# SUTD-MDQS/QILaplace.jl

Measured on AMD Instinct MI355X. Metric: MPO×MPS site-contractions/sec + max |coeff err|, n=24 χ_s=64 χ_c=128, higher is better.
Workload: dtype f64; 1 GPU; zt_n24_chi64_D128; sites=48, mps_bonds_max=64, mpo_bonds_max=128, parallelism=replicas x1 (one signal per GPU), ranks_reported_by_collective_backend=1

## Files before the change

### qilaplace.jl_amd/csrc/qil_internal.h

```cpp
#pragma once

#include <hip/hip_runtime.h>
#include <hip/hip_complex.h>

#include <cstdint>
#include <cstdio>
#include <cstring>
#include <functional>
#include <map>
#include <condition_variable>
#include <mutex>
#include <set>
#include <string>
#include <vector>

#include "qilaplace_hip.h"
#include "qilaplace_hip_testing.h"

#include <atomic>

struct qil_lds_grant {
    static constexpr int kDevices = 64;
    std::atomic<size_t> bytes[kDevices] = {};
    hipError_t ensure(int device, const void* fn, size_t want) {
// ... 145 lines not shown
        if (ctx) ctx->chains.erase(this);
    }
    int64_t n() const { return (int64_t)site.size(); }
    int64_t site_elems(int64_t i) const {
        return dims[i] * (phys_rank == 1 ? 2 : 4) * dims[i + 1];
    }
    size_t site_bytes(int64_t i) const { return (size_t)site_elems(i) * qil_elem_size(dtype); }
};
struct qil_mps : qil_chain {};
struct qil_mpo : qil_chain {};

int qil_chain_alloc(qil_context* ctx, qil_chain* c, int64_t n, int dtype, int paired, int phys_rank,
                    const int64_t* bond_dims, const int64_t* site_ids);
int qil_chain_release(qil_chain* c);
void qil_chain_bind(qil_chain* c, qil_context* ctx);
int qil_chain_set_site(qil_chain* c, int64_t i, void* p, int64_t dl, int64_t dr);
void qil_chain_adopt(qil_chain* c, int64_t i, void* p);

unsigned qil_fail_count();
struct qil_call_scope {
    qil_context* ctx;
    uint64_t serial0;
    unsigned fails0;
    explicit qil_call_scope(qil_context* c);
    ~qil_call_scope();
    qil_call_scope(const qil_call_scope&) = delete;
    qil_call_scope& operator=(const qil_call_scope&) = delete;
};

int qil_dev_right_envs(const struct qil_mps* psi, const char* verb, void** Rall, std::vector<long long>& roff, double* log_norm2);

int qil_dev_gemm(qil_context* ctx, int dtype, int opA, int opB, int64_t m, int64_t n, int64_t k,
                 const void* A, int64_t lda, const void* B, int64_t ldb, void* C, int64_t ldc);
int qil_dev_gemm_skinny(qil_context* ctx, int dtype, int opA, int opB, int64_t m, int64_t n, int64_t k,
                        const void* A, int64_t lda, const void* B, int64_t ldb, void* C, int64_t ldc);
struct qil_gemm_batch {
    int64_t count = 1;
    int64_t a_bs = 0, b_bs = 0, c_bs = 0;
    const uint8_t* b_sel = nullptr;
    int64_t b_sel_step = 0, b_sel_stride = 0;
};
int qil_dev_gemm_batched(qil_context* ctx, int dtype, int opA, int opB, int64_t m, int64_t n, int64_t k,
                         const void* A, int64_t lda, const void* B, int64_t ldb, void* C, int64_t ldc,
                         const qil_gemm_batch* batch);
struct qil_gemm_problem {
    const void* A;
    const void* B;
    void* C;
    int m, n, k;
    int lda, ldb, ldc;
    int tile_begin;
    int pad;
};
int qil_dev_gemm_grouped(qil_context* ctx, int dtype, std::vector<qil_gemm_problem>& probs);
bool qil_dev_gemm_grouped_fits(size_t nproblems);
int qil_check_pair(const char* verb, const struct qil_mps* phi, const struct qil_mps* psi);
int qil_sum_compress_impl(qil_context* ctx, const struct qil_mps* const* terms, int64_t nb, const double* w, int odt,
                          int64_t maxdim, double tol, int sweeps, int64_t zip_maxdim, struct qil_mps** out);
int qil_dev_diag_abs2(qil_context* ctx, int dtype, const void* R, int64_t ldr, int64_t n, double* host_out);
int qil_dev_transpose(qil_context* ctx, int dtype, int conj, int64_t m, int64_t n, const void* A, int64_t lda,
                      void* At, int64_t ldt);
int qil_dev_svd(qil_context* ctx, int dtype, int64_t m, int64_t n, void* A, int64_t lda, void* U,
                int64_t ldu, double* S_host, void* Vh, int64_t ldvh, double negligible_rel = 0.0);
int qil_dev_svd_left(qil_context* ctx, int dtype, int64_t p, int64_t q, void* B, int64_t ldb, void* Uiso, int64_t ldu,
                     double* S_host, void* SVh, int64_t ldsvh, double negligible_rel, int* handled, double cert_cutoff = 0.0,
                     double deflate = 0.0);
int qil_dev_qr_certified(qil_context* ctx, int dtype, int64_t m, int64_t n, const void* A, int64_t lda, double cutoff, void* Qout,
                         void* Rout, bool* certified);
// ... 14 lines not shown
```

### qilaplace.jl_amd/csrc/qil_linalg.hip

```cpp
#include <algorithm>
#include <chrono>
#include <cmath>
#include <cstring>
#include <numeric>
#include <utility>

#include "qil_internal.h"
#include "qil_launch.h"
#include "qil_device_utils.h"

namespace {

using namespace qil_dev;

constexpr int GK = 16;
#ifndef QIL_GEMM_GAUSS
#define QIL_GEMM_GAUSS 1
#endif
#ifndef QIL_GEMM_PAD
#define QIL_GEMM_PAD 2
#endif
constexpr int GPAD = QIL_GEMM_PAD;
typedef double d4 __attribute__((ext_vector_type(4)));

__device__ __forceinline__ void put_plane(double* S0, double* S1, int off, double v) {
    S0[off] = v;
    (void)S1;
}
__device__ __forceinline__ void put_plane(double* S0, double* S1, int off, c64 v) {
    S0[off] = v.re;
    S1[off] = v.im;
}
__device__ __forceinline__ double maybe_conj(double v, int) { return v; }
__device__ __forceinline__ c64 maybe_conj(c64 v, int cj) { return cj ? c64{v.re, -v.im} : v; }

template <class T, int BM, int BN, int WM, int WN, bool PIPE, bool ARC, bool BKC, int GKT = GK, int DEEP = 0>
__device__ __forceinline__ void gemm_mfma_body(const uint3 blockIdx, const uint3 gridDim, long long m, long long n, long long k_total,
                                                 const T* __restrict__ A, long long a_rs, long long a_ks, int conjA,
                                                 const T* __restrict__ B, long long b_ks, long long b_cs, int conjB,
                                                 T* __restrict__ C, long long ldc, long long kchunk,
                                                 long long cstride, int tiles_m, int tiles_n, int col_fastest,
                                                 long long a_bs, long long b_bs, long long c_bs,
                                                 const int* __restrict__ cmap, int cmap_blk,
                                                 const uint8_t* __restrict__ b_sel, long long b_sel_step,
                                                 long long b_sel_stride, int subtract) {
    constexpr bool CX = sizeof(T) == 16;
    constexpr int NP = CX ? 2 : 1;
    constexpr int LA = BM + GPAD, LB = BN + GPAD;
    constexpr int NBUF = PIPE ? 2 : 1;
    constexpr int TM = WM / 16, TN = WN / 16;
    constexpr int EA = BM * GKT / 256, EB = BN * GKT / 256;
    static_assert((BM / WM) * (BN / WN) == 4, "4 waves per workgroup");
    extern __shared__ __attribute__((aligned(16))) char gemm_smem[];
    double* As = reinterpret_cast<double*>(gemm_smem);
    double* Bs = As + NBUF * NP * GKT * LA;
    const int tid = threadIdx.x;
    const int lane = tid & 63, wave = tid >> 6;
    const int wr = (wave % (BM / WM)) * WM, wc = (wave / (BM / WM)) * WN;
    const int l15 = lane & 15, l4 = lane >> 4;
    int tile = blockIdx.x;
    if (col_fastest & 2) tile = (tile % 8) * (tiles_m * tiles_n / 8) + tile / 8;
    int tm, tn;
    if (col_fastest & 1) {
        tn = tile % tiles_n;
        tm = tile / tiles_n;
    } else {
        tm = tile % tiles_m;
        tn = tile / tiles_m;
    }
    const long long row0 = (long long)tm * BM, col0 = (long long)tn * BN;
    const long long kbeg = (long long)blockIdx.z * kchunk;
    const long long kend = min(k_total, kbeg + kchunk);
    A += (long long)blockIdx.y * a_bs;
    B += (long long)blockIdx.y * b_bs;
    if (b_sel) B += (long long)b_sel[(long long)blockIdx.y * b_sel_step] * b_sel_stride;
    C += (long long)blockIdx.z * cstride + (long long)blockIdx.y * c_bs;
    if (cmap) cmap += (long long)blockIdx.y * (n / cmap_blk);

    d4 rr[TM][TN], ii[CX ? TM : 1][CX ? TN : 1], ri[CX ? TM : 1][CX ? TN : 1];
#pragma unroll
    for (int a = 0; a < TM; ++a)
#pragma unroll
        for (int b = 0; b < TN; ++b) {
            rr[a][b] = d4{0, 0, 0, 0};
            if (CX) {
                ii[a][b] = d4{0, 0, 0, 0};
                ri[a][b] = d4{0, 0, 0, 0};
            }
        }
    constexpr bool a_rows_contig = ARC, b_k_contig = BKC;
    T ra[EA], rb[EB];
    const T* pa[EA];
    const T* pb[EB];
    int ka[EA], kb[EB], sa[EA], sb[EB];
#pragma unroll
    for (int e = 0; e < EA; ++e) {
        const int idx = tid + 256 * e;
        const int i = a_rows_contig ? idx % BM : idx / GKT;
        const int kk = a_rows_contig ? idx / BM : idx % GKT;
        const long long gr = row0 + i;
        ka[e] = kk;
        sa[e] = kk * LA + i;
        pa[e] = A + min(gr, m - 1) * a_rs + (kbeg + kk) * a_ks;
    }
#pragma unroll
    for (int e = 0; e < EB; ++e) {
        const int idx = tid + 256 * e;
        const int kk = b_k_contig ? idx % GKT : idx / BN;
        const int j = b_k_contig ? idx / GKT : idx % BN;
        const long long gc = col0 + j;
// ... 10 lines not shown
                pa[e] += a_step;
            }
#pragma unroll
            for (int e = 0; e < EB; ++e) {
                rb[e] = *pb[e];
                pb[e] += b_step;
            }
        } else {
#pragma unroll
            for (int e = 0; e < EA; ++e) ra[e] = *((k0 + ka[e] < kend) ? pa[e] : A);
#pragma unroll
            for (int e = 0; e < EB; ++e) rb[e] = *((k0 + kb[e] < kend) ? pb[e] : B);
        }
    };
    auto load_tile = [&](long long k0) { load_tile_into(ra, rb, k0); };
    auto store_tile_from = [&](const T(&ra)[EA], const T(&rb)[EB], int buf, long long k0) {
        double* a0 = As + (buf * NP) * GKT * LA;
        double* b0 = Bs + (buf * NP) * GKT * LB;
        if (k0 + GKT <= kend) {
#pragma unroll
            for (int e = 0; e < EA; ++e) put_plane(a0, a0 + GKT * LA, sa[e], maybe_conj(ra[e], conjA));
#pragma unroll
            for (int e = 0; e < EB; ++e) put_plane(b0, b0 + GKT * LB, sb[e], maybe_conj(rb[e], conjB));
        } else {
#pragma unroll
            for (int e = 0; e < EA; ++e)
                put_plane(a0, a0 + GKT * LA, sa[e], (k0 + ka[e] < kend) ? maybe_conj(ra[e], conjA) : T{});
#pragma unroll
            for (int e = 0; e < EB; ++e)
                put_plane(b0, b0 + GKT * LB, sb[e], (k0 + kb[e] < kend) ? maybe_conj(rb[e], conjB) : T{});
        }
    };
    auto store_tile = [&](int buf, long long k0) { store_tile_from(ra, rb, buf, k0); };
    auto mfma_tile = [&](int buf) {
        const double* a0 = As + (buf * NP) * GKT * LA;
        const double* b0 = Bs + (buf * NP) * GKT * LB;
#pragma unroll
        for (int kk = 0; kk < GKT; kk += 4) {
            double are[TM], aim[TM], bre[TN], bim[TN];
#pragma unroll
            for (int t = 0; t < TM; ++t) {
                are[t] = a0[(kk + l4) * LA + wr + 16 * t + l15];
                if (CX) aim[t] = a0[GKT * LA + (kk + l4) * LA + wr + 16 * t + l15];
            }
#pragma unroll
            for (int t = 0; t < TN; ++t) {
                bre[t] = b0[(kk + l4) * LB + wc + 16 * t + l15];
                if (CX) bim[t] = b0[GKT * LB + (kk + l4) * LB + wc + 16 * t + l15];
            }
            if constexpr (CX && QIL_GEMM_GAUSS) {
                double asum[TM], bsum[TN], bdif[TN];
#pragma unroll
                for (int t = 0; t < TM; ++t) asum[t] = are[t] + aim[t];
#pragma unroll
                for (int t = 0; t < TN; ++t) {
                    bsum[t] = bre[t] + bim[t];
                    bdif[t] = bim[t] - bre[t];
                }
#pragma unroll
                for (int ti = 0; ti < TM; ++ti)
#pragma unroll
                    for (int tj = 0; tj < TN; ++tj) {
                        rr[ti][tj] = __builtin_amdgcn_mfma_f64_16x16x4f64(bre[tj], asum[ti], rr[ti][tj], 0, 0, 0);
                        ii[ti][tj] = __builtin_amdgcn_mfma_f64_16x16x4f64(bsum[tj], aim[ti], ii[ti][tj], 0, 0, 0);
                        ri[ti][tj] = __builtin_amdgcn_mfma_f64_16x16x4f64(bdif[tj], are[ti], ri[ti][tj], 0, 0, 0);
                    }
            } else {
#pragma unroll
                for (int ti = 0; ti < TM; ++ti)
#pragma unroll
                    for (int tj = 0; tj < TN; ++tj) {
                        rr[ti][tj] = __builtin_amdgcn_mfma_f64_16x16x4f64(bre[tj], are[ti], rr[ti][tj], 0, 0, 0);
                        if constexpr (CX) {
                            ii[ti][tj] = __builtin_amdgcn_mfma_f64_16x16x4f64(bim[tj], aim[ti], ii[ti][tj], 0, 0, 0);
                            ri[ti][tj] = __builtin_amdgcn_mfma_f64_16x16x4f64(bim[tj], are[ti], ri[ti][tj], 0, 0, 0);
                            ri[ti][tj] = __builtin_amdgcn_mfma_f64_16x16x4f64(bre[tj], aim[ti], ri[ti][tj], 0, 0, 0);
                        }
                    }
            }
        }
    };
    if constexpr (PIPE && DEEP) {
        T ra1[EA], rb1[EB];
        if (kbeg < kend) load_tile_into(ra, rb, kbeg);
        if (kbeg + GKT < kend) load_tile_into(ra1, rb1, kbeg + GKT);
        for (long long k0 = kbeg; k0 < kend; k0 += 2 * GKT) {
            store_tile_from(ra, rb, 0, k0);
            __syncthreads();
            if (k0 + 2 * GKT < kend) load_tile_into(ra, rb, k0 + 2 * GKT);
            mfma_tile(0);
            if (k0 + GKT >= kend) break;
            store_tile_from(ra1, rb1, 1, k0 + GKT);
            __syncthreads();
            if (k0 + 3 * GKT < kend) load_tile_into(ra1, rb1, k0 + 3 * GKT);
            mfma_tile(1);
        }
    } else {
        int buf = 0;
        if (PIPE && kbeg < kend) load_tile(kbeg);
        for (long long k0 = kbeg; k0 < kend; k0 += GKT) {
            if (!PIPE) {
                if (k0 > kbeg) __syncthreads();
                load_tile(k0);
            }
            store_tile(buf, k0);
            __syncthreads();
            if (PIPE && k0 + GKT < kend) load_tile(k0 + GKT);
            mfma_tile(buf);
            if (PIPE) buf ^= 1;
        }
    }
#pragma unroll
    for (int ti = 0; ti < TM; ++ti)
#pragma unroll
        for (int tj = 0; tj < TN; ++tj)
#pragma unroll
            for (int r = 0; r < 4; ++r) {
                const long long gr = row0 + wr + 16 * ti + l15;
                const long long gc = col0 + wc + 16 * tj + l4 + 4 * r;
                if (gr < m && gc < n) {
                    const long long oc = cmap ? (long long)cmap[gc / cmap_blk] * cmap_blk + gc % cmap_blk : gc;
                    double* cp = reinterpret_cast<double*>(C + gr + ldc * oc);
                    if (subtract) {
                        if (CX) {
                            cp[0] -= rr[ti][tj][r] - ii[ti][tj][r];
                            cp[1] -= QIL_GEMM_GAUSS ? rr[ti][tj][r] + ri[ti][tj][r] : ri[ti][tj][r];
                        } else {
                            cp[0] -= rr[ti][tj][r];
                        }
                    } else if (CX) {
                        cp[0] = rr[ti][tj][r] - ii[ti][tj][r];
                        cp[1] = QIL_GEMM_GAUSS ? rr[ti][tj][r] + ri[ti][tj][r] : ri[ti][tj][r];
                    } else {
                        cp[0] = rr[ti][tj][r];
                    }
                }
            }
}
template <class T, int BM, int BN, int WM, int WN, bool PIPE, bool ARC, bool BKC, int GKT = GK, int DEEP = 0>
struct gemm_mfma_k {
    static constexpr int NT = 256, MINW = (DEEP ? 1 : (BM * BN <= 128 * 128 ? 2 : 1));
    template <class... QA>
    static __device__ __forceinline__ void run(const uint3 b, const uint3 g, QA... a) {
        gemm_mfma_body<T, BM, BN, WM, WN, PIPE, ARC, BKC, GKT, DEEP>(b, g, a...);
    }
};

template <class T>
__device__ __forceinline__ void splitk_reduce_body(const uint3 blockIdx, const uint3 gridDim, const T* __restrict__ W, long long cstride, int splits, long long m, long long n,
                              T* __restrict__ C, long long ldc, int subtract) {
    for (long long t = blockIdx.x * (long long)blockDim.x + threadIdx.x; t < m * n;
         t += (long long)gridDim.x * blockDim.x) {
        T acc = W[t];
        for (int z = 1; z < splits; ++z) acc = add_t(acc, W[t + z * cstride]);
        T* cp = C + (t % m) + ldc * (t / m);
        *cp = subtract ? sub_t(*cp, acc) : acc;
    }
}
template <class T>
struct splitk_reduce_k {
    static constexpr int NT = 1024, MINW = 1;
    template <class... QA>
    static __device__ __forceinline__ void run(const uint3 b, const uint3 g, QA... a) {
        splitk_reduce_body<T>(b, g, a...);
    }
};

struct gemm_batch {
    int count = 1;
    long long a_bs = 0, b_bs = 0, c_bs = 0;
    const int* cmap = nullptr;
    int cmap_blk = 1;
    const uint8_t* b_sel = nullptr;
    long long b_sel_step = 0, b_sel_stride = 0;
    int subtract = 0;
    int skinny_m = 0;
};

struct gemm_shape {
    int bm, bn, wm, wn, gkt, deep;
};
enum { GS_32x64_DEEP, GS_48x64_DEEP, GS_32x32, GS_64x64, GS_64x144, GS_128x128, GS_128x64, GS_COUNT };
constexpr gemm_shape GEMM_SHAPES[GS_COUNT] = {
    {32, 64, 16, 32, GK, 1}, {48, 64, 48, 16, GK, 1}, {32, 32, 16, 16, 32, 0}, {64, 64, 32, 32, GK, 0},
    {64, 144, 16, 144, GK, 0}, {128, 128, 64, 64, GK, 0}, {128, 64, 64, 32, GK, 0}};

int gemm_pick_shape(bool cx, long long m, long long n, long long count, int skinny_m) {
    if (skinny_m && m <= 32 && n >= 128) return GS_32x64_DEEP;
    if (skinny_m && m <= 48 && n >= 128) return GS_48x64_DEEP;
    constexpr long long small_tiles = 64;
    if (((m + 63) / 64) * ((n + 63) / 64) * count <= small_tiles && m >= 32 && n >= 32) return GS_32x32;
    if (cx) return GS_64x64;
    if (m >= 256 && n > 96 && n <= 144) return GS_64x144;
    {
        const long long t128 = ((m + 127) / 128) * ((n + 127) / 128);
        const bool fills = (double)m * (double)n >= 0.85 * 16384.0 * (double)t128;
        if (t128 * count >= 512 && fills) return GS_128x128;
    }
    {
        constexpr long long min_tiles = 128;
        const long long t = ((m + 127) / 128) * ((n + 63) / 64) * count;
        if (m >= 256 && t >= min_tiles) return GS_128x64;
    }
    return GS_64x64;
}

int gemm_plan(bool cx, int opA, int opB, long long m, long long n, long long k, long long lda, long long ldb, long long ldc,
              long long count, long long c_bs, bool has_cmap, int skinny_m, qil_gemm_plan_info* p) {
    const int si = gemm_pick_shape(cx, m, n, count, skinny_m);
    const gemm_shape& s = GEMM_SHAPES[si];
    p->bm = s.bm, p->bn = s.bn, p->wm = s.wm, p->wn = s.wn, p->gkt = s.gkt, p->deep = s.deep;
    const bool at = opA == 1 || opA == 2, bt = opB == 1 || opB == 2;
    p->arc = (at ? lda : 1) == 1;
    p->bkc = (bt ? ldb : 1) == 1;
    const long long tiles_m = (m + s.bm - 1) / s.bm, tiles_n = (n + s.bn - 1) / s.bn;
    const long long tiles = tiles_m * tiles_n;
    p->tiles_m = tiles_m, p->tiles_n = tiles_n;
    const bool can_split = count == 1 || (ldc == m && c_bs == m * n && !has_cmap);
    p->can_split = can_split;
    int splits = 1, rule = 0;
    static const long long split_min_k = 1024;
    if (can_split && tiles * count < 128 && (k >= split_min_k || (k >= 512 && tiles * count <= 8))) {
        splits = (int)std::min<long long>(std::min<long long>(k / 256, 512 / (tiles * count)), 64);
        rule = 1;
    }
    if (can_split && tiles * count <= 4 && k >= 128) {
        const int s2 = (int)std::min<long long>(k / 64, 32);
        if (s2 > splits) splits = s2, rule = 2;
    }
    if (splits < 2 && can_split && tiles * count >= 128 && tiles * count <= 384 && k >= 4096) {
        splits = (int)std::min<long long>(4, (767 / (tiles * count)));
        rule = 3;
    }
    if (splits < 2) splits = 1, rule = 0;
    long long kchunk = k;
    if (splits > 1) {
        kchunk = (((k + splits - 1) / splits) + s.gkt - 1) / s.gkt * s.gkt;
        splits = (int)((k + kchunk - 1) / kchunk);
    }
    p->splits = splits, p->split_rule = rule, p->kchunk = kchunk;
    p->col_fastest = tiles_n <= 8 ? 1 : 0;
    p->xcd = tiles >= 64 && tiles % 8 == 0;
    return si;
}

template <class T, int SI>
int gemm_launch(qil_context* ctx, const qil_gemm_plan_info& p, long long m, long long n, long long k, const T* A, long long a_rs,
                long long a_ks, int conjA, const T* B, long long b_ks, long long b_cs, int conjB, T* C,
                long long ldc, const gemm_batch& bt) {
    constexpr gemm_shape S = GEMM_SHAPES[SI];
    constexpr int BM = S.bm, BN = S.bn, WM = S.wm, WN = S.wn, GKT = S.gkt, DEEP = S.deep;
    constexpr bool PIPE = true;
    constexpr int NP = sizeof(T) == 16 ? 2 : 1;
    constexpr size_t lds = (size_t)(PIPE ? 2 : 1) * NP * GKT * ((BM + GPAD) + (BN + GPAD)) * sizeof(double);
    const long long tiles = p.tiles_m * p.tiles_n;
    const int splits = p.splits;
    long long cstride = 0, c_bs = bt.c_bs;
    T* Cout = C;
    long long ldo = ldc;
    void* wsp = nullptr;
    if (splits > 1) {
        cstride = m * n * bt.count;
        c_bs = m * n;
        QIL_TRY(qil_ctx_alloc(ctx, (size_t)(cstride * splits) * sizeof(T), &wsp));
        Cout = static_cast<T*>(wsp);
        ldo = m;
    }
    const int order = p.col_fastest | (p.xcd ? 2 : 0);
#define QIL_GEMM_K(ARCv, BKCv)                                                                                               \
    QIL_TRY((qil_klaunch<gemm_mfma_k<T, BM, BN, WM, WN, PIPE, ARCv, BKCv, GKT, DEEP>>(                                                      \
        ctx, dim3((unsigned)tiles, (unsigned)bt.count, (unsigned)splits), dim3(256), lds, m, n, k, A, a_rs, a_ks, conjA, B, b_ks, \
        b_cs, conjB, Cout, ldo, (long long)p.kchunk, cstride, (int)p.tiles_m, (int)p.tiles_n, order, bt.a_bs, bt.b_bs, c_bs, bt.cmap,  \
        bt.cmap_blk, bt.b_sel, bt.b_sel_step, bt.b_sel_stride, splits > 1 ? 0 : bt.subtract)))
    if (p.arc && p.bkc) QIL_GEMM_K(true, true);
    else if (p.arc) QIL_GEMM_K(true, false);
    else if (p.bkc) QIL_GEMM_K(false, true);
    else QIL_GEMM_K(false, false);
#undef QIL_GEMM_K
    if (splits > 1) {
        QIL_TRY((qil_klaunch<splitk_reduce_k<T>>(ctx, dim3((unsigned)std::min<long long>((cstride + 255) / 256, 2048)), dim3(256), 0, (const T*)Cout, cstride, splits, m, n * bt.count, C, ldc, bt.subtract)));
        QIL_HIP(hipGetLastError());
        qil_ctx_free(ctx, wsp);
    }
    return QIL_OK;
}

template <class T>
int gemm_dispatch(qil_context* ctx, int opA, int opB, long long m, long long n, long long k, const T* A,
                  long long lda, const T* B, long long ldb, T* C, long long ldc,
                  const gemm_batch& batch = gemm_batch{}) {
    if (m == 0 || n == 0) return QIL_OK;
    QIL_REQUIRE(opA >= 0 && opA <= 3 && opB >= 0 && opB <= 3, QIL_EINVAL_ARG, "gemm: bad op codes %d, %d", opA, opB);
    const bool at = opA == 1 || opA == 2, bt = opB == 1 || opB == 2;
    const long long a_rs = at ? lda : 1, a_ks = at ? 1 : lda;
    const long long b_ks = bt ? ldb : 1, b_cs = bt ? 1 : ldb;
    const int cA = (opA == 2 || opA == 3) ? 1 : 0, cB = (opB == 2 || opB == 3) ? 1 : 0;
    constexpr bool CX = sizeof(T) == 16;
    qil_gemm_plan_info p;
    const int si = gemm_plan(CX, opA, opB, m, n, k, lda, ldb, ldc, batch.count, batch.c_bs, batch.cmap != nullptr, batch.skinny_m, &p);
#define QIL_GEMM_GO(SI) \
    case SI: return gemm_launch<T, SI>(ctx, p, m, n, k, A, a_rs, a_ks, cA, B, b_ks, b_cs, cB, C, ldc, batch)
    switch (si) {
        QIL_GEMM_GO(GS_32x64_DEEP);
        QIL_GEMM_GO(GS_48x64_DEEP);
        QIL_GEMM_GO(GS_32x32);
        QIL_GEMM_GO(GS_64x64);
    }
    if constexpr (!CX) {
        switch (si) {
            QIL_GEMM_GO(GS_64x144);
            QIL_GEMM_GO(GS_128x128);
            QIL_GEMM_GO(GS_128x64);
        }
    }
#undef QIL_GEMM_GO
    return qil_fail(QIL_EINVAL_ARG, "gemm: no kernel for tile shape %d", si);
}

template <class T>
__device__ __forceinline__ void jacobi_round_body(const uint3 blockIdx, const uint3 gridDim, T* __restrict__ A, long long lda, long long m,
                                                    T* __restrict__ V, long long ldv, int vrows, int n,
                                                    int npad, int round, double tol,
                                                    int* __restrict__ rotated,
                                                    const double* __restrict__ negligible) {
    __shared__ double red[16];
    const int i = blockIdx.x;
    int p, q;
    if (i == 0) {
        p = npad - 1;
        q = round;
    } else {
        p = (round + i) % (npad - 1);
// ... 3560 lines not shown
    }
}
template <class T>
struct scale_kernel_k {
    static constexpr int NT = 1024, MINW = 1;
    template <class... QA>
    static __device__ __forceinline__ void run(const uint3 b, const uint3 g, QA... a) {
        scale_kernel_body<T>(b, g, a...);
    }
};

__global__ void fill_normal_kernel(double* __restrict__ p, long long n, uint64_t seed, double scale) {
    for (long long t = blockIdx.x * (long long)blockDim.x + threadIdx.x; t < n;
         t += (long long)gridDim.x * blockDim.x) {
        const uint64_t h1 = splitmix64(seed ^ splitmix64(2ull * (uint64_t)t));
        const uint64_t h2 = splitmix64(seed ^ splitmix64(2ull * (uint64_t)t + 1ull));
        const double u1 = ((double)(h1 >> 11) + 1.0) * (1.0 / 9007199254740993.0);
        const double u2 = (double)(h2 >> 11) * (1.0 / 9007199254740992.0);
        p[t] = scale * sqrt(-2.0 * log(u1)) * cospi(2.0 * u2);
    }
}

}

int qil_dev_gemm(qil_context* ctx, int dtype, int opA, int opB, int64_t m, int64_t n, int64_t k,
                 const void* A, int64_t lda, const void* B, int64_t ldb, void* C, int64_t ldc) {
    if (dtype == QIL_C64)
        return gemm_dispatch<c64>(ctx, opA, opB, m, n, k, (const c64*)A, lda, (const c64*)B, ldb, (c64*)C, ldc);
    static const int real_op[4] = {0, 1, 1, 0};
    return gemm_dispatch<double>(ctx, real_op[opA & 3], real_op[opB & 3], m, n, k, (const double*)A, lda,
                                 (const double*)B, ldb, (double*)C, ldc);
}

int qil_dev_gemm_skinny(qil_context* ctx, int dtype, int opA, int opB, int64_t m, int64_t n, int64_t k,
                        const void* A, int64_t lda, const void* B, int64_t ldb, void* C, int64_t ldc) {
    gemm_batch bt;
    bt.skinny_m = 1;
    if (dtype == QIL_C64)
        return gemm_dispatch<c64>(ctx, opA, opB, m, n, k, (const c64*)A, lda, (const c64*)B, ldb, (c64*)C, ldc, bt);
    static const int real_op[4] = {0, 1, 1, 0};
    return gemm_dispatch<double>(ctx, real_op[opA & 3], real_op[opB & 3], m, n, k, (const double*)A, lda,
                                 (const double*)B, ldb, (double*)C, ldc, bt);
}

static int gemm_check_args(int opA, int opB, int64_t m, int64_t n, int64_t k, int64_t lda, int64_t ldb, int64_t ldc) {
    QIL_REQUIRE(m >= 1 && n >= 1 && k >= 1, QIL_EINVAL_ARG, "gemm: empty operand");
    QIL_REQUIRE(opA >= 0 && opA <= 3 && opB >= 0 && opB <= 3, QIL_EINVAL_ARG, "gemm: bad op code");
    const int64_t a_rows = (opA == 0 || opA == 3) ? m : k, b_rows = (opB == 0 || opB == 3) ? k : n;
    QIL_REQUIRE(lda >= a_rows, QIL_EINVAL_ARG, "gemm: lda %lld is smaller than the %lld stored rows of A", (long long)lda, (long long)a_rows);
    QIL_REQUIRE(ldb >= b_rows, QIL_EINVAL_ARG, "gemm: ldb %lld is smaller than the %lld stored rows of B", (long long)ldb, (long long)b_rows);
    QIL_REQUIRE(ldc >= m, QIL_EINVAL_ARG, "gemm: ldc %lld is smaller than the %lld rows of C", (long long)ldc, (long long)m);
    return QIL_OK;
}

extern "C" int qil_gemm(qil_context* ctx, int dtype, int opA, int opB, int64_t m, int64_t n, int64_t k,
                        const void* A, int64_t lda, const void* B, int64_t ldb, void* C, int64_t ldc) {
    QIL_REQUIRE(ctx && A && B && C, QIL_EINVAL_ARG, "gemm: null argument");
    QIL_TRY(gemm_check_args(opA, opB, m, n, k, lda, ldb, ldc));
    QIL_TRY(qil_ctx_activate(ctx));
    qil_call_scope call_scope(ctx);
    const size_t e = qil_elem_size(dtype);
    const int64_t a_cols = (opA == 0 || opA == 3) ? k : m, b_cols = (opB == 0 || opB == 3) ? n : k;
    void *dA = nullptr, *dB = nullptr, *dC = nullptr;
    QIL_TRY(qil_ctx_alloc(ctx, (size_t)(lda * a_cols) * e, &dA));
    QIL_TRY(qil_ctx_alloc(ctx, (size_t)(ldb * b_cols) * e, &dB));
    QIL_TRY(qil_ctx_alloc(ctx, (size_t)(ldc * n) * e, &dC));
    QIL_HIP(hipMemcpyAsync(dA, A, (size_t)(lda * a_cols) * e, hipMemcpyHostToDevice, qil_stream(ctx)));
    QIL_HIP(hipMemcpyAsync(dB, B, (size_t)(ldb * b_cols) * e, hipMemcpyHostToDevice, qil_stream(ctx)));
    QIL_TRY(qil_dev_zero(ctx, dC, (size_t)(ldc * n) * e));
    QIL_HIP(qil_stream_sync(ctx));
    QIL_TRY(qil_dev_gemm(ctx, dtype, opA, opB, m, n, k, dA, lda, dB, ldb, dC, ldc));
    QIL_TRY(qil_read_back(ctx, C, dC, (size_t)(ldc * n) * e));
    qil_ctx_free(ctx, dA);
    qil_ctx_free(ctx, dB);
    qil_ctx_free(ctx, dC);
// ... 330 lines not shown
```

### qilaplace.jl_amd/csrc/qil_readout.hip

```cpp
#include "qil_internal.h"
#include "qil_launch.h"
#include "qil_device_utils.h"
#include <set>
#include <mutex>
#include <map>

namespace {

using namespace qil_dev;

__device__ __forceinline__ double shfl_xor_t(double v, int m) { return __shfl_xor(v, m, 64); }
__device__ __forceinline__ c64 shfl_xor_t(c64 v, int m) {
    return c64{__shfl_xor(v.re, m, 64), __shfl_xor(v.im, m, 64)};
}
__device__ __forceinline__ double one_t(double) { return 1.0; }
__device__ __forceinline__ c64 one_t(c64) { return c64{1.0, 0.0}; }

struct ChainSite {
    const void* A;
    const void* W;
    int cl, cr, Dl, Dr;
};

constexpr int kThreads = 256;
// ... 92 lines not shown
}

template <class T>
__global__ void select_slice(const T* __restrict__ Tm, long long nb, int cr, const uint8_t* __restrict__ bits,
                             int n, int site, T* __restrict__ Vn) {
    const long long total = nb * cr;
    for (long long t = blockIdx.x * (long long)blockDim.x + threadIdx.x; t < total;
         t += (long long)gridDim.x * blockDim.x) {
        const long long q = t % nb;
        const long long beta = t / nb;
        const int bit = bits[q * n + site];
        Vn[t] = bit == 2 ? add_t(Tm[q + nb * (2 * beta)], Tm[q + nb * (1 + 2 * beta)])
                         : Tm[q + nb * (bit + 2 * beta)];
    }
}

template <class T>
__device__ __forceinline__ void select_slice_body(const uint3 blockIdx, const uint3 gridDim, const T* __restrict__ Tm, long long nb, int cr,
                                                  const uint8_t* __restrict__ bits, int n, int site, T* __restrict__ Vn) {
    const long long total = nb * cr;
    for (long long t = blockIdx.x * (long long)blockDim.x + threadIdx.x; t < total; t += (long long)gridDim.x * blockDim.x) {
        const long long q = t % nb;
        const long long beta = t / nb;
        const int bit = bits[q * n + site];
        Vn[t] = bit == 2 ? add_t(Tm[q + nb * (2 * beta)], Tm[q + nb * (1 + 2 * beta)]) : Tm[q + nb * (bit + 2 * beta)];
    }
}
template <class T>
struct select_slice_k {
    static constexpr int NT = 256, MINW = 1;
    template <class... QA>
    static __device__ __forceinline__ void run(const uint3 b, const uint3 g, QA... a) {
        select_slice_body<T>(b, g, a...);
    }
};
template <class T>
__device__ __forceinline__ void gather_rows_body(const uint3 blockIdx, const uint3 gridDim, const T* __restrict__ Tm, long long nb, int cr,
                                                 const int* __restrict__ map, T* __restrict__ Vn) {
    const long long total = nb * cr;
    for (long long t = blockIdx.x * (long long)blockDim.x + threadIdx.x; t < total; t += (long long)gridDim.x * blockDim.x) {
        const long long r = t % nb, beta = t / nb;
        Vn[t] = Tm[map[r] + nb * beta];
    }
}
template <class T>
struct gather_rows_k {
    static constexpr int NT = 256, MINW = 1;
    template <class... QA>
    static __device__ __forceinline__ void run(const uint3 b, const uint3 g, QA... a) {
        gather_rows_body<T>(b, g, a...);
    }
};
template <class T>
__device__ __forceinline__ void fill_ones_body(const uint3 blockIdx, const uint3 gridDim, T* __restrict__ v, long long n) {
    for (long long t = blockIdx.x * (long long)blockDim.x + threadIdx.x; t < n; t += (long long)gridDim.x * blockDim.x) v[t] = one_t(T{});
}
template <class T>
struct fill_ones_k {
    static constexpr int NT = 256, MINW = 1;
    template <class... QA>
    static __device__ __forceinline__ void run(const uint3 b, const uint3 g, QA... a) {
        fill_ones_body<T>(b, g, a...);
    }
};
template <class T>
__device__ __forceinline__ void finish_coeff_body(const uint3 blockIdx, const uint3 gridDim, const T* __restrict__ v, long long nb,
                                                  double amplitude, c64* __restrict__ out) {
    for (long long t = blockIdx.x * (long long)blockDim.x + threadIdx.x; t < nb; t += (long long)gridDim.x * blockDim.x) {
        const c64 r = to_c64(v[t]);
        out[t] = c64{r.re * amplitude, r.im * amplitude};
    }
}
template <class T>
struct finish_coeff_k {
    static constexpr int NT = 256, MINW = 1;
    template <class... QA>
    static __device__ __forceinline__ void run(const uint3 b, const uint3 g, QA... a) {
        finish_coeff_body<T>(b, g, a...);
    }
};

template <class T>
__global__ void fill_ones(T* __restrict__ v, long long n) {
// ... 146 lines not shown

int upload_bits(qil_context* ctx, int64_t nb, int64_t n, const uint8_t* bits, uint8_t** dbits, int max_bit = 1) {
    for (int64_t t = 0; t < nb * n; ++t)
        QIL_REQUIRE(bits[t] <= max_bit, QIL_EINVAL_CONFIG, "coefficient: bit value %d outside [0,%d]", (int)bits[t],
                    max_bit);
    void* p = nullptr;
    QIL_TRY(qil_ctx_alloc(ctx, (size_t)(nb * n), &p));
    hipError_t e = hipMemcpyAsync(p, bits, (size_t)(nb * n), hipMemcpyHostToDevice, qil_stream(ctx));
    if (e == hipSuccess) e = qil_stream_sync(ctx);
    if (e != hipSuccess) {
        qil_ctx_free(ctx, p);
        return qil_fail(QIL_EHIP, "bit upload failed: %s", hipGetErrorString(e));
    }
    *dbits = static_cast<uint8_t*>(p);
    return QIL_OK;
}

}

static int coefficient_impl(const qil_mps* psi, int64_t nb, const uint8_t* bits, double* out, int max_bit);

extern "C" int qil_coefficient_batch(const qil_mps* psi, int64_t nb, const uint8_t* bits, double* out) {
    return coefficient_impl(psi, nb, bits, out, 1);
}

extern "C" int qil_coefficient_marginal_batch(const qil_mps* psi, int64_t nb, const uint8_t* bits, double* out) {
    return coefficient_impl(psi, nb, bits, out, 2);
}

struct SortPlan {
    int* dmap = nullptr;
    std::vector<int64_t> n0;
};
static int build_sort_plan(qil_context* ctx, int64_t nb, int64_t n, const uint8_t* bits, SortPlan* plan) {
    std::vector<int> map((size_t)(n * nb)), order((size_t)nb), next((size_t)nb), pos((size_t)nb);
    plan->n0.assign((size_t)n, 0);
    auto order_of = [&](int64_t site, std::vector<int>& o) -> int64_t {
        int64_t z = 0;
        if (site >= n) {
            for (int64_t q = 0; q < nb; ++q) o[(size_t)q] = (int)q;
            return nb;
        }
        for (int64_t q = 0; q < nb; ++q)
            if (bits[q * n + site] == 0) o[(size_t)z++] = (int)q;
        int64_t w = z;
        for (int64_t q = 0; q < nb; ++q)
            if (bits[q * n + site] != 0) o[(size_t)w++] = (int)q;
        return z;
    };
    plan->n0[0] = order_of(0, order);
    for (int64_t i = 0; i < n; ++i) {
        for (int64_t r = 0; r < nb; ++r) pos[(size_t)order[(size_t)r]] = (int)r;
        const int64_t z = order_of(i + 1, next);
        if (i + 1 < n) plan->n0[(size_t)i + 1] = z;
        for (int64_t r = 0; r < nb; ++r) map[(size_t)(i * nb + r)] = pos[(size_t)next[(size_t)r]];
        order.swap(next);
    }
    void* p = nullptr;
    QIL_TRY(qil_ctx_alloc(ctx, map.size() * sizeof(int), &p));
    hipError_t e = hipMemcpyAsync(p, map.data(), map.size() * sizeof(int), hipMemcpyHostToDevice, qil_stream(ctx));
    if (e == hipSuccess) e = qil_stream_sync(ctx);
    if (e != hipSuccess) {
        qil_ctx_free(ctx, p);
        return qil_fail(QIL_EHIP, "read-out plan upload failed: %s", hipGetErrorString(e));
    }
    plan->dmap = static_cast<int*>(p);
    return QIL_OK;
}
static bool wants_sort_plan(const qil_mps* psi, int64_t nb, int max_bit) {
    if (max_bit > 1 || nb < 4) return false;
    long long maxchi = 1;
    for (int64_t i = 0; i < psi->n(); ++i) maxchi = std::max<long long>(maxchi, psi->dims[(size_t)i + 1]);
    return maxchi >= 128 || (nb >= 1024 && maxchi >= 16);
}

static int coefficient_enqueue(const qil_mps* psi, int64_t nb, const uint8_t* dbits, void* dout, const SortPlan* plan = nullptr) {
    qil_context* ctx = psi->ctx;
    const int64_t n = psi->n();
    std::vector<ChainSite> tab((size_t)n);
    long long maxchi = 1;
    for (int64_t i = 0; i < n; ++i) {
        tab[(size_t)i] = ChainSite{psi->site[(size_t)i], nullptr, (int)psi->dims[(size_t)i],
                                   (int)psi->dims[(size_t)i + 1], 1, 1};
        maxchi = std::max<long long>(maxchi, psi->dims[(size_t)i + 1]);
    }
    const size_t esz = qil_elem_size(psi->dtype);
    static const long long min_chi = 128;
    if (nb >= 4 && (maxchi >= min_chi || (nb >= 1024 && maxchi >= 16))) {
        void *V = nullptr, *Vn = nullptr, *Tm = nullptr;
        QIL_TRY(qil_ctx_alloc(ctx, (size_t)(nb * maxchi) * esz, &V));
        QIL_TRY(qil_ctx_alloc(ctx, (size_t)(nb * maxchi) * esz, &Vn));
        QIL_TRY(qil_ctx_alloc(ctx, (size_t)(2 * nb * maxchi) * esz, &Tm));
        const bool cx = psi->dtype == QIL_C64;
        const unsigned g1 = (unsigned)std::min<long long>((nb + 255) / 256, 4096);
        if (cx) QIL_TRY((qil_klaunch<fill_ones_k<c64>>(ctx, dim3(g1), dim3(256), 0, (c64*)V, (long long)nb)));
        else QIL_TRY((qil_klaunch<fill_ones_k<double>>(ctx, dim3(g1), dim3(256), 0, (double*)V, (long long)nb)));
        for (int64_t i = 0; i < n; ++i) {
            const int64_t cl = psi->dims[(size_t)i], cr = psi->dims[(size_t)i + 1];
            const unsigned g = (unsigned)std::min<long long>((nb * cr + 255) / 256, 65536);
            if (plan && plan->dmap) {
                const int64_t z = plan->n0[(size_t)i];
                const char* site = static_cast<const char*>(psi->site[(size_t)i]);
                for (int sl = 0; sl < 2; ++sl) {
                    const int64_t r0 = sl ? z : 0, rows = sl ? nb - z : z;
                    if (rows == 0) continue;
                    const void* Vs = static_cast<const char*>(V) + (size_t)r0 * esz;
                    void* Ts = static_cast<char*>(Tm) + (size_t)r0 * esz;
                    const void* As = site + (size_t)(sl * cl) * esz;
                    if (rows <= 48) QIL_TRY(qil_dev_gemm_skinny(ctx, psi->dtype, 0, 0, rows, cr, cl, Vs, nb, As, 2 * cl, Ts, nb));
                    else QIL_TRY(qil_dev_gemm(ctx, psi->dtype, 0, 0, rows, cr, cl, Vs, nb, As, 2 * cl, Ts, nb));
                }
                const int* map = plan->dmap + (size_t)(i * nb);
                if (cx) QIL_TRY((qil_klaunch<gather_rows_k<c64>>(ctx, dim3(g), dim3(256), 0, (const c64*)Tm, (long long)nb, (int)cr, map, (c64*)Vn)));
                else QIL_TRY((qil_klaunch<gather_rows_k<double>>(ctx, dim3(g), dim3(256), 0, (const double*)Tm, (long long)nb, (int)cr, map, (double*)Vn)));
                std::swap(V, Vn);
                continue;
            }
            QIL_TRY(qil_dev_gemm(ctx, psi->dtype, 0, 0, nb, 2 * cr, cl, V, nb, psi->site[(size_t)i], cl, Tm, nb));
            if (cx)
                QIL_TRY((qil_klaunch<select_slice_k<c64>>(ctx, dim3(g), dim3(256), 0, (const c64*)Tm, (long long)nb, (int)cr,
                                                          (const uint8_t*)dbits, (int)n, (int)i, (c64*)Vn)));
            else
                QIL_TRY((qil_klaunch<select_slice_k<double>>(ctx, dim3(g), dim3(256), 0, (const double*)Tm, (long long)nb, (int)cr,
                                                             (const uint8_t*)dbits, (int)n, (int)i, (double*)Vn)));
            std::swap(V, Vn);
        }
        if (cx) QIL_TRY((qil_klaunch<finish_coeff_k<c64>>(ctx, dim3(g1), dim3(256), 0, (const c64*)V, (long long)nb, psi->amplitude, (c64*)dout)));
        else QIL_TRY((qil_klaunch<finish_coeff_k<double>>(ctx, dim3(g1), dim3(256), 0, (const double*)V, (long long)nb, psi->amplitude, (c64*)dout)));
        qil_ctx_free(ctx, V);
        qil_ctx_free(ctx, Vn);
        qil_ctx_free(ctx, Tm);
        return QIL_OK;
    }
    void *scratch = nullptr, *pin = nullptr, *dtab = nullptr;
    int slot = 0;
    QIL_TRY(qil_ctx_alloc(ctx, (size_t)(2 * nb * maxchi) * esz, &scratch));
    QIL_TRY(qil_ctx_desc_acquire(ctx, tab.size() * sizeof(ChainSite), &pin, &dtab, &slot));
    memcpy(pin, tab.data(), tab.size() * sizeof(ChainSite));
    QIL_HIP(hipMemcpyAsync(dtab, pin, tab.size() * sizeof(ChainSite), hipMemcpyHostToDevice, qil_stream(ctx)));
    if (psi->dtype == QIL_C64)
        hipLaunchKernelGGL(coefficient_chain<c64>, dim3((unsigned)nb), dim3(kThreads), 0, qil_stream(ctx),
                           (const ChainSite*)dtab, (int)n, dbits, (c64*)scratch, maxchi, (c64*)dout,
                           psi->amplitude);
    else
        hipLaunchKernelGGL(coefficient_chain<double>, dim3((unsigned)nb), dim3(kThreads), 0, qil_stream(ctx),
                           (const ChainSite*)dtab, (int)n, dbits, (double*)scratch, maxchi, (c64*)dout,
                           psi->amplitude);
    QIL_HIP(hipGetLastError());
    QIL_TRY(qil_ctx_desc_commit(ctx, slot));
    qil_ctx_free(ctx, scratch);
    return QIL_OK;
}

static int coefficient_impl(const qil_mps* psi, int64_t nb, const uint8_t* bits, double* out, int max_bit) {
    QIL_REQUIRE(psi && (nb == 0 || (bits && out)), QIL_EINVAL_ARG, "coefficient: null argument");
    if (nb == 0) return QIL_OK;
    qil_context* ctx = psi->ctx;
    QIL_TRY(qil_ctx_activate(ctx));
    qil_call_scope call_scope(ctx);
    uint8_t* dbits = nullptr;
    QIL_TRY(upload_bits(ctx, nb, psi->n(), bits, &dbits, max_bit));
    SortPlan plan;
    if (wants_sort_plan(psi, nb, max_bit)) QIL_TRY(build_sort_plan(ctx, nb, psi->n(), bits, &plan));
    void* dout = nullptr;
// ... 232 lines not shown
```

Baseline: 3862 site-contractions/s.

## Fuse sorted-readout row gather into GEMM epilogue via row map and batched halves

```diff
diff --git a/qilaplace.jl_amd/csrc/qil_internal.h b/qilaplace.jl_amd/csrc/qil_internal.h
--- a/qilaplace.jl_amd/csrc/qil_internal.h
+++ b/qilaplace.jl_amd/csrc/qil_internal.h
@@ -201,8 +201,8 @@
 
 int qil_dev_gemm(qil_context* ctx, int dtype, int opA, int opB, int64_t m, int64_t n, int64_t k,
                  const void* A, int64_t lda, const void* B, int64_t ldb, void* C, int64_t ldc);
-int qil_dev_gemm_skinny(qil_context* ctx, int dtype, int opA, int opB, int64_t m, int64_t n, int64_t k,
-                        const void* A, int64_t lda, const void* B, int64_t ldb, void* C, int64_t ldc);
+int qil_dev_gemm_rows(qil_context* ctx, int dtype, int64_t m0, int64_t m1, int64_t n, int64_t k, const void* A, int64_t lda,
+                      const void* B, int64_t ldb, int64_t b_step, void* C, int64_t ldc, const int* rmap);
 struct qil_gemm_batch {
     int64_t count = 1;
     int64_t a_bs = 0, b_bs = 0, c_bs = 0;
diff --git a/qilaplace.jl_amd/csrc/qil_linalg.hip b/qilaplace.jl_amd/csrc/qil_linalg.hip
--- a/qilaplace.jl_amd/csrc/qil_linalg.hip
+++ b/qilaplace.jl_amd/csrc/qil_linalg.hip
@@ -3,6 +3,7 @@
 #include <cmath>
 #include <cstring>
 #include <numeric>
+#include <type_traits>
 #include <utility>
 
 #include "qil_internal.h"
@@ -34,6 +35,10 @@
 __device__ __forceinline__ double maybe_conj(double v, int) { return v; }
 __device__ __forceinline__ c64 maybe_conj(c64 v, int cj) { return cj ? c64{v.re, -v.im} : v; }
 
+struct gemm_row_step {
+    int rmap_bs, m_step;
+};
+
 template <class T, int BM, int BN, int WM, int WN, bool PIPE, bool ARC, bool BKC, int GKT = GK, int DEEP = 0>
 __device__ __forceinline__ void gemm_mfma_body(const uint3 blockIdx, const uint3 gridDim, long long m, long long n, long long k_total,
                                                  const T* __restrict__ A, long long a_rs, long long a_ks, int conjA,
@@ -42,9 +47,11 @@
                                                  long long cstride, int tiles_m, int tiles_n, int col_fastest,
                                                  long long a_bs, long long b_bs, long long c_bs,
                                                  const int* __restrict__ cmap, int cmap_blk,
+                                                 const int* __restrict__ rmap, gemm_row_step rows,
                                                  const uint8_t* __restrict__ b_sel, long long b_sel_step,
-                                                 long long b_sel_stride, int subtract) {
+                                                 long long b_sel_stride) {
     constexpr bool CX = sizeof(T) == 16;
+    const int subtract = col_fastest & 4;
     constexpr int NP = CX ? 2 : 1;
     constexpr int LA = BM + GPAD, LB = BN + GPAD;
     constexpr int NBUF = PIPE ? 2 : 1;
@@ -76,6 +83,12 @@
     if (b_sel) B += (long long)b_sel[(long long)blockIdx.y * b_sel_step] * b_sel_stride;
     C += (long long)blockIdx.z * cstride + (long long)blockIdx.y * c_bs;
     if (cmap) cmap += (long long)blockIdx.y * (n / cmap_blk);
+    m += (long long)blockIdx.y * rows.m_step;
+    if (rmap) rmap += (long long)blockIdx.y * rows.rmap_bs;
+    if (row0 >= m) return;
+    int nact = TM;
+    if constexpr (DEEP != 0)
+        nact = (int)max(0LL, min((long long)TM, (m - row0 - __builtin_amdgcn_readfirstlane(wr) + 15) / 16));
 
     d4 rr[TM][TN], ii[CX ? TM : 1][CX ? TN : 1], ri[CX ? TM : 1][CX ? TN : 1];
 #pragma unroll
@@ -152,14 +165,15 @@
         }
     };
     auto store_tile = [&](int buf, long long k0) { store_tile_from(ra, rb, buf, k0); };
-    auto mfma_tile = [&](int buf) {
+    auto mfma_rows = [&](int buf, auto na) {
+        constexpr int NA = decltype(na)::value;
         const double* a0 = As + (buf * NP) * GKT * LA;
         const double* b0 = Bs + (buf * NP) * GKT * LB;
 #pragma unroll
         for (int kk = 0; kk < GKT; kk += 4) {
-            double are[TM], aim[TM], bre[TN], bim[TN];
-#pragma unroll
-            for (int t = 0; t < TM; ++t) {
+            double are[NA], aim[NA], bre[TN], bim[TN];
+#pragma unroll
+            for (int t = 0; t < NA; ++t) {
                 are[t] = a0[(kk + l4) * LA + wr + 16 * t + l15];
                 if (CX) aim[t] = a0[GKT * LA + (kk + l4) * LA + wr + 16 * t + l15];
             }
@@ -169,16 +183,16 @@
                 if (CX) bim[t] = b0[GKT * LB + (kk + l4) * LB + wc + 16 * t + l15];
             }
             if constexpr (CX && QIL_GEMM_GAUSS) {
-                double asum[TM], bsum[TN], bdif[TN];
-#pragma unroll
-                for (int t = 0; t < TM; ++t) asum[t] = are[t] + aim[t];
+                double asum[NA], bsum[TN], bdif[TN];
+#pragma unroll
+                for (int t = 0; t < NA; ++t) asum[t] = are[t] + aim[t];
 #pragma unroll
                 for (int t = 0; t < TN; ++t) {
                     bsum[t] = bre[t] + bim[t];
                     bdif[t] = bim[t] - bre[t];
                 }
 #pragma unroll
-                for (int ti = 0; ti < TM; ++ti)
+                for (int ti = 0; ti < NA; ++ti)
 #pragma unroll
                     for (int tj = 0; tj < TN; ++tj) {
                         rr[ti][tj] = __builtin_amdgcn_mfma_f64_16x16x4f64(bre[tj], asum[ti], rr[ti][tj], 0, 0, 0);
@@ -187,7 +201,7 @@
                     }
             } else {
 #pragma unroll
-                for (int ti = 0; ti < TM; ++ti)
+                for (int ti = 0; ti < NA; ++ti)
 #pragma unroll
                     for (int tj = 0; tj < TN; ++tj) {
                         rr[ti][tj] = __builtin_amdgcn_mfma_f64_16x16x4f64(bre[tj], are[ti], rr[ti][tj], 0, 0, 0);
@@ -198,6 +212,15 @@
                         }
                     }
             }
+        }
+    };
+    auto mfma_tile = [&](int buf) {
+        if constexpr (DEEP != 0) {
+            if (nact == TM) mfma_rows(buf, std::integral_constant<int, TM>{});
+            else if (TM > 2 && nact == 2) mfma_rows(buf, std::integral_constant<int, (TM > 2 ? 2 : 1)>{});
+            else if (TM > 1 && nact == 1) mfma_rows(buf, std::integral_constant<int, 1>{});
+        } else {
+            mfma_rows(buf, std::integral_constant<int, TM>{});
         }
     };
     if constexpr (PIPE && DEEP) {
@@ -240,7 +263,8 @@
                 const long long gc = col0 + wc + 16 * tj + l4 + 4 * r;
                 if (gr < m && gc < n) {
                     const long long oc = cmap ? (long long)cmap[gc / cmap_blk] * cmap_blk + gc % cmap_blk : gc;
-                    double* cp = reinterpret_cast<double*>(C + gr + ldc * oc);
+                    const long long orow = rmap ? (long long)rmap[gr] : gr;
+                    double* cp = reinterpret_cast<double*>(C + orow + ldc * oc);
                     if (subtract) {
                         if (CX) {
                             cp[0] -= rr[ti][tj][r] - ii[ti][tj][r];
@@ -268,12 +292,12 @@
 
 template <class T>
 __device__ __forceinline__ void splitk_reduce_body(const uint3 blockIdx, const uint3 gridDim, const T* __restrict__ W, long long cstride, int splits, long long m, long long n,
-                              T* __restrict__ C, long long ldc, int subtract) {
+                              T* __restrict__ C, long long ldc, int subtract, const int* __restrict__ rmap) {
     for (long long t = blockIdx.x * (long long)blockDim.x + threadIdx.x; t < m * n;
          t += (long long)gridDim.x * blockDim.x) {
         T acc = W[t];
         for (int z = 1; z < splits; ++z) acc = add_t(acc, W[t + z * cstride]);
-        T* cp = C + (t % m) + ldc * (t / m);
+        T* cp = C + (rmap ? (long long)rmap[t % m] : t % m) + ldc * (t / m);
         *cp = subtract ? sub_t(*cp, acc) : acc;
     }
 }
@@ -291,6 +315,8 @@
     long long a_bs = 0, b_bs = 0, c_bs = 0;
     const int* cmap = nullptr;
     int cmap_blk = 1;
+    const int* rmap = nullptr;
+    long long rmap_bs = 0, m_step = 0;
     const uint8_t* b_sel = nullptr;
     long long b_sel_step = 0, b_sel_stride = 0;
     int subtract = 0;
@@ -326,7 +352,7 @@
 }
 
 int gemm_plan(bool cx, int opA, int opB, long long m, long long n, long long k, long long lda, long long ldb, long long ldc,
-              long long count, long long c_bs, bool has_cmap, int skinny_m, qil_gemm_plan_info* p) {
+              long long count, long long c_bs, bool has_cmap, int skinny_m, qil_gemm_plan_info* p, bool has_rmap = false) {
     const int si = gemm_pick_shape(cx, m, n, count, skinny_m);
     const gemm_shape& s = GEMM_SHAPES[si];
     p->bm = s.bm, p->bn = s.bn, p->wm = s.wm, p->wn = s.wn, p->gkt = s.gkt, p->deep = s.deep;
@@ -336,7 +362,7 @@
     const long long tiles_m = (m + s.bm - 1) / s.bm, tiles_n = (n + s.bn - 1) / s.bn;
     const long long tiles = tiles_m * tiles_n;
     p->tiles_m = tiles_m, p->tiles_n = tiles_n;
-    const bool can_split = count == 1 || (ldc == m && c_bs == m * n && !has_cmap);
+    const bool can_split = count == 1 || has_rmap || (ldc == m && c_bs == m * n && !has_cmap);
     p->can_split = can_split;
     int splits = 1, rule = 0;
     static const long long split_min_k = 1024;
@@ -379,26 +405,38 @@
     T* Cout = C;
     long long ldo = ldc;
     void* wsp = nullptr;
+    const int* rmap = bt.rmap;
+    const long long mt = m + (bt.count - 1) * (bt.rmap_bs + bt.m_step);
     if (splits > 1) {
-        cstride = m * n * bt.count;
-        c_bs = m * n;
+        if (rmap) {
+            cstride = mt * n;
+            c_bs = bt.rmap_bs;
+            ldo = mt;
+            rmap = nullptr;
+        } else {
+            cstride = m * n * bt.count;
+            c_bs = m * n;
+            ldo = m;
+        }
         QIL_TRY(qil_ctx_alloc(ctx, (size_t)(cstride * splits) * sizeof(T), &wsp));
         Cout = static_cast<T*>(wsp);
-        ldo = m;
-    }
-    const int order = p.col_fastest | (p.xcd ? 2 : 0);
+    }
+    const int order = p.col_fastest | (p.xcd ? 2 : 0) | (splits == 1 && bt.subtract ? 4 : 0);
 #define QIL_GEMM_K(ARCv, BKCv)                                                                                               \
     QIL_TRY((qil_klaunch<gemm_mfma_k<T, BM, BN, WM, WN, PIPE, ARCv, BKCv, GKT, DEEP>>(                                                      \
         ctx, dim3((unsigned)tiles, (unsigned)bt.count, (unsigned)splits), dim3(256), lds, m, n, k, A, a_rs, a_ks, conjA, B, b_ks, \
         b_cs, conjB, Cout, ldo, (long long)p.kchunk, cstride, (int)p.tiles_m, (int)p.tiles_n, order, bt.a_bs, bt.b_bs, c_bs, bt.cmap,  \
-        bt.cmap_blk, bt.b_sel, bt.b_sel_step, bt.b_sel_stride, splits > 1 ? 0 : bt.subtract)))
+        bt.cmap_blk, rmap, gemm_row_step{(int)bt.rmap_bs, (int)bt.m_step}, bt.b_sel, bt.b_sel_step, bt.b_sel_stride)))
     if (p.arc && p.bkc) QIL_GEMM_K(true, true);
     else if (p.arc) QIL_GEMM_K(true, false);
     else if (p.bkc) QIL_GEMM_K(false, true);
     else QIL_GEMM_K(false, false);
 #undef QIL_GEMM_K
     if (splits > 1) {
-        QIL_TRY((qil_klaunch<splitk_reduce_k<T>>(ctx, dim3((unsigned)std::min<long long>((cstride + 255) / 256, 2048)), dim3(256), 0, (const T*)Cout, cstride, splits, m, n * bt.count, C, ldc, bt.subtract)));
+        if (bt.rmap)
+            QIL_TRY((qil_klaunch<splitk_reduce_k<T>>(ctx, dim3((unsigned)std::min<long long>((cstride + 255) / 256, 2048)), dim3(256), 0, (const T*)Cout, cstride, splits, mt, n, C, ldc, bt.subtract, bt.rmap)));
+        else
+            QIL_TRY((qil_klaunch<splitk_reduce_k<T>>(ctx, dim3((unsigned)std::min<long long>((cstride + 255) / 256, 2048)), dim3(256), 0, (const T*)Cout, cstride, splits, m, n * bt.count, C, ldc, bt.subtract, (const int*)nullptr)));
         QIL_HIP(hipGetLastError());
         qil_ctx_free(ctx, wsp);
     }
@@ -417,7 +455,11 @@
     const int cA = (opA == 2 || opA == 3) ? 1 : 0, cB = (opB == 2 || opB == 3) ? 1 : 0;
     constexpr bool CX = sizeof(T) == 16;
     qil_gemm_plan_info p;
-    const int si = gemm_plan(CX, opA, opB, m, n, k, lda, ldb, ldc, batch.count, batch.c_bs, batch.cmap != nullptr, batch.skinny_m, &p);
+    const long long mp = std::max(m, m + (batch.count - 1) * batch.m_step);
+    QIL_REQUIRE(!batch.rmap || (!batch.cmap && batch.c_bs == 0), QIL_EINVAL_ARG, "gemm: a row map excludes a column map and a C stride");
+    QIL_REQUIRE(batch.m_step == 0 || (batch.rmap && m + (batch.count - 1) * batch.m_step >= 1), QIL_EINVAL_ARG, "gemm: bad row step %lld", batch.m_step);
+    const int si = gemm_plan(CX, opA, opB, mp, n, k, lda, ldb, ldc, batch.count, batch.c_bs, batch.cmap != nullptr, batch.skinny_m, &p,
+                             batch.rmap != nullptr);
 #define QIL_GEMM_GO(SI) \
     case SI: return gemm_launch<T, SI>(ctx, p, m, n, k, A, a_rs, a_ks, cA, B, b_ks, b_cs, cB, C, ldc, batch)
     switch (si) {
@@ -4044,15 +4086,20 @@
                                  (const double*)B, ldb, (double*)C, ldc);
 }
 
-int qil_dev_gemm_skinny(qil_context* ctx, int dtype, int opA, int opB, int64_t m, int64_t n, int64_t k,
-                        const void* A, int64_t lda, const void* B, int64_t ldb, void* C, int64_t ldc) {
+int qil_dev_gemm_rows(qil_context* ctx, int dtype, int64_t m0, int64_t m1, int64_t n, int64_t k, const void* A, int64_t lda,
+                      const void* B, int64_t ldb, int64_t b_step, void* C, int64_t ldc, const int* rmap) {
+    QIL_REQUIRE(m0 >= 1 && m1 >= 0 && rmap, QIL_EINVAL_ARG, "gemm_rows: bad row blocks %lld, %lld", (long long)m0, (long long)m1);
     gemm_batch bt;
-    bt.skinny_m = 1;
+    bt.rmap = rmap;
+    bt.skinny_m = std::max(m0, m1) <= 48;
+    if (m1 > 0) {
+        QIL_REQUIRE(bt.skinny_m, QIL_EINVAL_ARG, "gemm_rows: two row blocks share a launch on the skinny tiles only");
+        bt.count = 2;
+        bt.a_bs = m0, bt.b_bs = b_step, bt.rmap_bs = m0, bt.m_step = m1 - m0;
+    }
     if (dtype == QIL_C64)
-        return gemm_dispatch<c64>(ctx, opA, opB, m, n, k, (const c64*)A, lda, (const c64*)B, ldb, (c64*)C, ldc, bt);
-    static const int real_op[4] = {0, 1, 1, 0};
-    return gemm_dispatch<double>(ctx, real_op[opA & 3], real_op[opB & 3], m, n, k, (const double*)A, lda,
-                                 (const double*)B, ldb, (double*)C, ldc, bt);
+        return gemm_dispatch<c64>(ctx, 0, 0, m0, n, k, (const c64*)A, lda, (const c64*)B, ldb, (c64*)C, ldc, bt);
+    return gemm_dispatch<double>(ctx, 0, 0, m0, n, k, (const double*)A, lda, (const double*)B, ldb, (double*)C, ldc, bt);
 }
 
 static int gemm_check_args(int opA, int opB, int64_t m, int64_t n, int64_t k, int64_t lda, int64_t ldb, int64_t ldc) {
diff --git a/qilaplace.jl_amd/csrc/qil_readout.hip b/qilaplace.jl_amd/csrc/qil_readout.hip
--- a/qilaplace.jl_amd/csrc/qil_readout.hip
+++ b/qilaplace.jl_amd/csrc/qil_readout.hip
@@ -148,23 +148,6 @@
     template <class... QA>
     static __device__ __forceinline__ void run(const uint3 b, const uint3 g, QA... a) {
         select_slice_body<T>(b, g, a...);
-    }
-};
-template <class T>
-__device__ __forceinline__ void gather_rows_body(const uint3 blockIdx, const uint3 gridDim, const T* __restrict__ Tm, long long nb, int cr,
-                                                 const int* __restrict__ map, T* __restrict__ Vn) {
-    const long long total = nb * cr;
-    for (long long t = blockIdx.x * (long long)blockDim.x + threadIdx.x; t < total; t += (long long)gridDim.x * blockDim.x) {
-        const long long r = t % nb, beta = t / nb;
-        Vn[t] = Tm[map[r] + nb * beta];
-    }
-}
-template <class T>
-struct gather_rows_k {
-    static constexpr int NT = 256, MINW = 1;
-    template <class... QA>
-    static __device__ __forceinline__ void run(const uint3 b, const uint3 g, QA... a) {
-        gather_rows_body<T>(b, g, a...);
     }
 };
 template <class T>
@@ -377,9 +360,10 @@
     int* dmap = nullptr;
     std::vector<int64_t> n0;
 };
-static int build_sort_plan(qil_context* ctx, int64_t nb, int64_t n, const uint8_t* bits, SortPlan* plan) {
-    std::vector<int> map((size_t)(n * nb)), order((size_t)nb), next((size_t)nb), pos((size_t)nb);
-    plan->n0.assign((size_t)n, 0);
+static void sort_plan_maps(int64_t nb, int64_t n, const uint8_t* bits, std::vector<int>& map, std::vector<int64_t>& n0) {
+    std::vector<int> order((size_t)nb), next((size_t)nb), pos((size_t)nb);
+    map.assign((size_t)(n * nb), 0);
+    n0.assign((size_t)n, 0);
     auto order_of = [&](int64_t site, std::vector<int>& o) -> int64_t {
         int64_t z = 0;
         if (site >= n) {
@@ -393,14 +377,18 @@
             if (bits[q * n + site] != 0) o[(size_t)w++] = (int)q;
         return z;
     };
-    plan->n0[0] = order_of(0, order);
+    n0[0] = order_of(0, order);
     for (int64_t i = 0; i < n; ++i) {
         for (int64_t r = 0; r < nb; ++r) pos[(size_t)order[(size_t)r]] = (int)r;
         const int64_t z = order_of(i + 1, next);
-        if (i + 1 < n) plan->n0[(size_t)i + 1] = z;
-        for (int64_t r = 0; r < nb; ++r) map[(size_t)(i * nb + r)] = pos[(size_t)next[(size_t)r]];
+        if (i + 1 < n) n0[(size_t)i + 1] = z;
+        for (int64_t r = 0; r < nb; ++r) map[(size_t)(i * nb + pos[(size_t)next[(size_t)r]])] = (int)r;
         order.swap(next);
     }
+}
+static int build_sort_plan(qil_context* ctx, int64_t nb, int64_t n, const uint8_t* bits, SortPlan* plan) {
+    std::vector<int> map;
+    sort_plan_maps(nb, n, bits, map, plan->n0);
     void* p = nullptr;
     QIL_TRY(qil_ctx_alloc(ctx, map.size() * sizeof(int), &p));
     hipError_t e = hipMemcpyAsync(p, map.data(), map.size() * sizeof(int), hipMemcpyHostToDevice, qil_stream(ctx));
@@ -432,10 +420,11 @@
     const size_t esz = qil_elem_size(psi->dtype);
     static const long long min_chi = 128;
     if (nb >= 4 && (maxchi >= min_chi || (nb >= 1024 && maxchi >= 16))) {
+        const bool sorted = plan && plan->dmap;
         void *V = nullptr, *Vn = nullptr, *Tm = nullptr;
         QIL_TRY(qil_ctx_alloc(ctx, (size_t)(nb * maxchi) * esz, &V));
         QIL_TRY(qil_ctx_alloc(ctx, (size_t)(nb * maxchi) * esz, &Vn));
-        QIL_TRY(qil_ctx_alloc(ctx, (size_t)(2 * nb * maxchi) * esz, &Tm));
+        if (!sorted) QIL_TRY(qil_ctx_alloc(ctx, (size_t)(2 * nb * maxchi) * esz, &Tm));
         const bool cx = psi->dtype == QIL_C64;
         const unsigned g1 = (unsigned)std::min<long long>((nb + 255) / 256, 4096);
         if (cx) QIL_TRY((qil_klaunch<fill_ones_k<c64>>(ctx, dim3(g1), dim3(256), 0, (c64*)V, (long long)nb)));
@@ -443,21 +432,21 @@
         for (int64_t i = 0; i < n; ++i) {
             const int64_t cl = psi->dims[(size_t)i], cr = psi->dims[(size_t)i + 1];
             const unsigned g = (unsigned)std::min<long long>((nb * cr + 255) / 256, 65536);
-            if (plan && plan->dmap) {
+            if (sorted) {
                 const int64_t z = plan->n0[(size_t)i];
                 const char* site = static_cast<const char*>(psi->site[(size_t)i]);
-                for (int sl = 0; sl < 2; ++sl) {
-                    const int64_t r0 = sl ? z : 0, rows = sl ? nb - z : z;
-                    if (rows == 0) continue;
-                    const void* Vs = static_cast<const char*>(V) + (size_t)r0 * esz;
-                    void* Ts = static_cast<char*>(Tm) + (size_t)r0 * esz;
-                    const void* As = site + (size_t)(sl * cl) * esz;
-                    if (rows <= 48) QIL_TRY(qil_dev_gemm_skinny(ctx, psi->dtype, 0, 0, rows, cr, cl, Vs, nb, As, 2 * cl, Ts, nb));
-                    else QIL_TRY(qil_dev_gemm(ctx, psi->dtype, 0, 0, rows, cr, cl, Vs, nb, As, 2 * cl, Ts, nb));
+                const int* map = plan->dmap + (size_t)(i * nb);
+                if (z > 0 && z < nb && std::max(z, nb - z) <= 48) {
+                    QIL_TRY(qil_dev_gemm_rows(ctx, psi->dtype, z, nb - z, cr, cl, V, nb, site, 2 * cl, cl, Vn, nb, map));
+                } else {
+                    for (int sl = 0; sl < 2; ++sl) {
+                        const int64_t r0 = sl ? z : 0, rows = sl ? nb - z : z;
+                        if (rows == 0) continue;
+                        const void* Vs = static_cast<const char*>(V) + (size_t)r0 * esz;
+                        const void* As = site + (size_t)(sl * cl) * esz;
+                        QIL_TRY(qil_dev_gemm_rows(ctx, psi->dtype, rows, 0, cr, cl, Vs, nb, As, 2 * cl, 0, Vn, nb, map + r0));
+                    }
                 }
-                const int* map = plan->dmap + (size_t)(i * nb);
-                if (cx) QIL_TRY((qil_klaunch<gather_rows_k<c64>>(ctx, dim3(g), dim3(256), 0, (const c64*)Tm, (long long)nb, (int)cr, map, (c64*)Vn)));
-                else QIL_TRY((qil_klaunch<gather_rows_k<double>>(ctx, dim3(g), dim3(256), 0, (const double*)Tm, (long long)nb, (int)cr, map, (double*)Vn)));
                 std::swap(V, Vn);
                 continue;
             }
@@ -474,7 +463,7 @@
         else QIL_TRY((qil_klaunch<finish_coeff_k<double>>(ctx, dim3(g1), dim3(256), 0, (const double*)V, (long long)nb, psi->amplitude, (c64*)dout)));
         qil_ctx_free(ctx, V);
         qil_ctx_free(ctx, Vn);
-        qil_ctx_free(ctx, Tm);
+        if (Tm) qil_ctx_free(ctx, Tm);
         return QIL_OK;
     }
     void *scratch = nullptr, *pin = nullptr, *dtab = nullptr;
```

New measurement: 3822 site-contractions/s. 1.0% lower.
